# timbroed/HRFuser

Measured on AMD Instinct MI355X. Metric: train images/sec HRFuser-T r640 3-modal @1/2/4/8 MI355X; fwd ms/img, higher is better.
Workload: dtype f32; 1 GPU; t_nus_bn backbone train step (fwd+bwd+grad exchange+AdamW at lr 0), 2 img/GPU, 2x3x384x640 camera + 2 modalities, BN, single GPU; global_batch=2, parallelism=dp1, launch=hipGraph replay

## Files before the change

hrfuser_amd/_lib.py:

```python
import ctypes
import os
import re

import torch

_HERE = os.path.dirname(os.path.abspath(__file__))
HEADER = os.path.join(os.path.dirname(_HERE), 'include', 'hrfuser_hip.h')
DEBUG_HEADER = os.path.join(os.path.dirname(_HERE), 'include', 'hrfuser_hip_debug.h')
LIB_PATH = os.environ.get('HRF_LIB_PATH') or os.path.join(_HERE, 'libhrfuser_hip.so')

def _header_int(name, default):
    m = re.search(r'#define\s+' + name + r'\s+(\d+)', open(HEADER).read())
    return int(m.group(1)) if m else default


STAT_COPIES = _header_int('HRF_STAT_COPIES', 16)
FIN_MAXC = _header_int('HRF_FIN_MAXC', 576)
C3X_MAXC = _header_int('HRF_C3X_MAXC', 256)

def struct_from_header(tag, path=HEADER):
    src = re.sub(r'/\*.*?\*/', '', open(path).read(), flags=re.S)
    m = re.search(r'typedef\s+struct\s+' + tag + r'\s*\{(.*?)\}\s*' + tag + r'_t\s*;', src, flags=re.S)
    if not m:
        raise KeyError(tag)
# ... 19 lines not shown
    return type(tag, (ctypes.Structure,), {'_fields_': fields})


BnFin = struct_from_header('hrf_bn_fin')
BnBFin = struct_from_header('hrf_bn_bfin')
AttnBlock = struct_from_header('hrf_attn_block')
FfnEval = struct_from_header('hrf_ffn_eval')
Conv3xPackJob = struct_from_header('hrf_conv3x_pack_job')
P2p = struct_from_header('hrf_p2p')


def _ptr(t):
    return None if t is None else t.data_ptr()


_RAW_RETURN = ('hrf_conv3_wgrad_wide_scratch', 'hrf_conv_bwd_weight_scratch', 'hrf_conv3x_pack_size', 'hrf_conv3x_supported', 'hrf_conv_fwd_split_scratch', 'hrf_wgrad_group_report', 'hrf_attn_block_supported', 'hrf_attn_block_bwd_supported', 'hrf_group_count',
               'hrf_ffn_eval_supported', 'hrf_get_deterministic', 'hrf_det_bins_bytes', 'hrf_conv3_bf16x3_supported')
_ERR = {1: 'HRF_ERR_ARG (bad argument)', 2: 'HRF_ERR_LAUNCH (kernel launch failed)'}


class HRFuserHipError(RuntimeError):
    pass


def parse_header(path=HEADER):
    src = open(path).read()
    src = re.sub(r'/\*.*?\*/', '', src, flags=re.S)
    protos = {}
    for m in re.finditer(r'\b(?:int|long)\s+(hrf_\w+)\s*\(([^)]*)\)\s*;', src):
        args = []
        for a in m.group(2).split(','):
# ... 103 lines not shown
```

hrfuser_amd/backbone.py:

```python
import os
import warnings

import torch
import torch.nn as nn

from . import _lib
from . import runtime as R
from .registry import BACKBONES

WIN = 7


def build_bn(norm_cfg, c):
    cfg = dict(norm_cfg or dict(type='BN'))
    kind = cfg.pop('type')
    if kind not in ('BN', 'SyncBN', 'GN'):
        raise KeyError(f'unsupported norm_cfg type {kind}')
    requires_grad = cfg.pop('requires_grad', True)
    if kind == 'GN':
        if 'num_groups' not in cfg:
            raise AssertionError('norm_cfg of type GN needs num_groups')
        bn = nn.GroupNorm(cfg['num_groups'], c, eps=cfg.get('eps', 1e-5))
    else:
        bn = nn.BatchNorm2d(c, eps=cfg.get('eps', 1e-5), momentum=cfg.get('momentum', 0.1))
# ... 147 lines not shown
            od += 4 * C * K
            of += 7 * C
            oc += C
        self._csum = csum
        self._rs0 = bns[0].running_mean.data_ptr() if (bns and bns[0].running_mean is not None) else 0
        if bns:
            self._gidx, self._bidx = torch.cat(gidx).to(device), torch.cat(bidx).to(device)
            self._epsv = torch.cat(epsv).to(device)
        offs = {id(p): o for p, (o, _) in zip(params, self._spans)}
        self._poffs = offs
        self.fs_layers, self.fs_sig = {}, None
        self.pslot, cols, ps = {}, [], 0
        for m in self.root.modules():
            hit = isinstance(m, nn.LayerNorm) or (isinstance(m, nn.Conv2d) and m.groups == m.in_channels and m.groups > 1)
            cand = (m.weight, m.bias) if hit else ()
            if hasattr(m, 'relative_position_bias_table'):
                cand = (m.relative_position_bias_table,) + tuple(
                    getattr(m, n).bias for n in ('qkv', 'k_proj', 'v_proj') if hasattr(m, n))
            for q in cand:
                if q is None or id(q) not in offs or id(q) in self.pslot:
                    continue
                self.pslot[id(q)] = ps
                cols.append(torch.arange(offs[id(q)], offs[id(q)] + q.numel(), dtype=torch.int32))
                ps += q.numel()
        self.ps_n = ps
        self.ps_map = (torch.cat(cols) if cols else torch.zeros(0, dtype=torch.int32)).to(device)
        self.ps_scratch = torch.zeros(max(1, K * ps), device=device, dtype=torch.float32)
        self.ps_dirty = False
        nbt = [m.num_batches_tracked for m in bns if m.num_batches_tracked is not None]
        self.nbt_flat = torch.zeros(len(nbt), device=device, dtype=torch.long)
# ... 1555 lines not shown
```

hrfuser_amd/csrc/conv_engine.hip:

```cpp
#include <algorithm>
#include <cstdlib>
#include <vector>
#include "hrf_common.h"
#include "hrf_group.h"
#include "hrf_lin.h"
#include "../../include/hrfuser_hip.h"

#include "hrf_wgrad.h"

namespace {

constexpr int BM = 64;
constexpr int BK = 64;
constexpr int LDK = 65;
constexpr float SENT = -1.0e30f;

static int g_knob[12] = {0, 0, 0, 0, 0, 0, 0, 0, 0, 0, 0, 0};

__device__ __forceinline__ float act_at_read(int tf, float u) {
  return tf == HRF_TF_AFFINE_RELU ? fmaxf(u, 0.f) : (tf == HRF_TF_AFFINE_GELU ? hrf_gelu(u) : u);
}

struct ConvFwdArgs {
  const float* x; const float* w; const float* bias;
// ... 922 lines not shown
  if (KH == 3 && stride == 2 && Cout >= (g_knob[5] > 0 ? g_knob[5] : 16) && sC == 1 && sY == W * sX && sB == H * sY && g_knob[6] == 0) {
    Conv3Args c{};
    c.in = dy + doff; c.ldIn = ldD; c.in2 = cA != nullptr ? yraw + doff : nullptr; c.t0 = cA; c.t1 = cB; c.t2 = cC;
    c.w = w; c.wCin = Cin; c.out = dx; c.ldOut = sX; c.accumulate = accumulate; c.epi = epi; c.xraw = xraw; c.ldXr = ldXr;
    c.esc = tf_scale; c.esh = tf_shift; c.act = act; c.stats = stats; c.bfin = a.bfin;
    c.B = B; c.H = H; c.W = W; c.Cin = Cout; c.Cout = Cin; c.Hs = a.Ho; c.Ws = a.Wo;
    return hrf_conv3s2_bwd_data_launch(c, stream);
  }
  const int nt = pick_nt(Cin);
  if (KH == 1) {
    if (cA != nullptr) { HRF_BD_NT(1, true) } else { HRF_BD_NT(1, false) }
  } else {
    if (cA != nullptr) { HRF_BD_NT(3, true) } else { HRF_BD_NT(3, false) }
  }
  return hrf_check_launch();
}

extern "C" int hrf_conv3x_supported(int Cin, int Cout, int KH, int stride, int dir) {
  if (KH != 3 || Cin <= 0 || Cout <= 0) return 0;
  if (dir == 0) return (stride == 1 || stride == 2) && Cout > 32 ? 1 : 0;
  if (stride == 2) return Cin > 32 && Cout <= 64 ? 1 : 0;
  return stride == 1 && Cin > 32 ? 1 : 0;
}

extern "C" int hrf_conv_fwd_packed(const float* x, int sB, int sY, int sX, int sC, int B, int H, int W, int Cin,
                                   const float* w, const float* bias, int KH, int stride, int Cout,
                                   float* y, int ldY, int yoff, const float* res, const float* res2, int ldR,
                                   int tf_mode, const float* tf_scale, const float* tf_shift,
                                   const float* tf_rowstat, double* stats, const hrf_bn_fin_t* tf_fin, float* ln_rowstat,
                                   float ln_eps, const float* wp, void* stream) {
// ... 335 lines not shown
```

hrfuser_amd/csrc/hrf_lin.h:

```cpp
#pragma once
#include "../../include/hrfuser_hip.h"

struct LinFwdArgs {
  const float* x; int ldX;
  const float* w; const float* bias;
  float* y; int ldY; int yoff;
  const float* res; const float* res2; int ldR;
  int tf_mode; const float* tf_scale; const float* tf_shift; const float* tf_rowstat;
  double* stats;
  float* ln_out; float ln_eps;
  hrf_bn_fin_t fin;
  int M, K, N;
};

struct LinBwdDataArgs {
  const float* dy; int ldD; int doff; const float* yraw;
  const float* cA; const float* cB; const float* cC;
  const float* w;
  float* dx; int ldDx; int accumulate;
  int epi; const float* xraw; int ldXr; const float* tf_scale; const float* tf_shift; int act;
  double* stats;
  hrf_bn_bfin_t bfin;
  int M, K, N;
};

int hrf_lin_fwd_launch(const LinFwdArgs& a, void* stream);
bool hrf_lin_fwd_emits_ln(const LinFwdArgs& a);
int hrf_lin_bwd_data_launch(const LinBwdDataArgs& a, void* stream);
int hrf_lin2_fwd_launch(const LinFwdArgs& a, void* stream);
bool hrf_lin2_fwd_emits_ln(const LinFwdArgs& a);
int hrf_lin2_bwd_data_launch(const LinBwdDataArgs& a, void* stream);

struct Conv3Args {
  const float* in; int ldIn;
  const float* in2;
  const float* t0; const float* t1; const float* t2;
  int tf_mode;
  const float* w; int wCin;
  const float* bias;
  float* out; int ldOut; int ooff;
  const float* res; const float* res2; int ldR;
  int accumulate, epi; const float* xraw; int ldXr; const float* esc; const float* esh; int act;
  double* stats;
  hrf_bn_fin_t fin;
  hrf_bn_bfin_t bfin;
  int B, H, W, Cin, Cout;
// ... 31 lines not shown
```

hrfuser_amd/csrc/lin2_engine.hip:

```cpp
#include <type_traits>
#include "hrf_common.h"
#include "hrf_lin.h"
#include "hrf_group.h"
#include "../../include/hrfuser_hip.h"

namespace {

constexpr int GK = 16, GLP = GK + 4, NW = 4, NTHR = 64 * NW, GROWS = 16 * NW;

template <int CG_, int CT_, int PD_>
struct Tile {
  static constexpr int CG = CG_, CT = CT_, PD = PD_;
  static constexpr int NB = CG * CT * 16, RT = CG, RG = NW / CG;
  static constexpr int SLOT = (GROWS + NB) * GLP;
  static constexpr int NWV = (NB * 4 + NTHR - 1) / NTHR;
  static constexpr int Q = CT * 4, PE = CT * 16 + 4, NRG = NTHR / Q, NR = (GROWS + NRG - 1) / NRG;
  static constexpr int RED = NRG * 2 * CT * 16;
  static_assert(GROWS * PE <= 2 * SLOT, "the transposed accumulator tile must fit the operand ring");
};
typedef Tile<1, 5, 4> TileA;
typedef Tile<2, 5, 4> TileB;
typedef Tile<2, 8, 2> TileC;
typedef Tile<2, 10, 2> TileD;

// ... 574 lines not shown

int hrf_lin2_fwd_launch(const LinFwdArgs& a, void* stream) {
  if (!wide_enough(a.M, a.K, a.N)) return -1;
  if (a.ln_out != nullptr && g_l2_knob[0] != 1) return -1;
  if ((long)a.M * a.ldX >= (1L << 32)) return -1;
  if (a.tf_mode != HRF_TF_NONE && a.tf_mode != HRF_TF_LN && a.fin.stats != nullptr && a.K > HRF_FIN_MAXC) return -1;
  const int id = pick_tile(a.N);
  switch (id) {
    case 1: return launch_fwd_tf<TileA>(a, id, stream);
    case 2: return launch_fwd_tf<TileB>(a, id, stream);
    case 3: return launch_fwd_tf<TileC>(a, id, stream);
    default: return launch_fwd_tf<TileD>(a, id, stream);
  }
}
bool hrf_lin2_fwd_emits_ln(const LinFwdArgs&) { return false; }
int hrf_lin2_bwd_data_launch(const LinBwdDataArgs& a, void* stream) {
  if (!wide_enough(a.M, a.K, a.N)) return -1;
  if (a.cA != nullptr && a.bfin.gstats != nullptr && a.K > HRF_FIN_MAXC) return -1;
  if ((long)a.M * a.ldD + a.doff >= (1L << 32)) return -1;
  const int id = pick_tile(a.N);
  switch (id) {
    case 1: return launch_bwd_b<TileA>(a, id, stream);
    case 2: return launch_bwd_b<TileB>(a, id, stream);
    case 3: return launch_bwd_b<TileC>(a, id, stream);
    default: return launch_bwd_b<TileD>(a, id, stream);
  }
}
#if defined(HRF_L2_TIMING) && !defined(HRF_EMUL)
extern "C" int hrf_lin2_stamps(long long* out) {
  return hipMemcpyFromSymbol(out, HIP_SYMBOL(g_l2_t), sizeof(long long) * 64) == hipSuccess ? HRF_OK : HRF_ERR_LAUNCH;
// ... 8 lines not shown
```

hrfuser_amd/csrc/lin_engine.hip:

```cpp
#include "hrf_common.h"
#include "hrf_lin.h"
#include "hrf_group.h"
#include "../../include/hrfuser_hip.h"

namespace {

#ifndef HRF_LIN_BWD_EPI_MAX_NT
#define HRF_LIN_BWD_EPI_MAX_NT 5
#endif
constexpr int LIN_BWD_EPI_MAX_NT = HRF_LIN_BWD_EPI_MAX_NT;
#ifndef HRF_LIN_FWD_MAX_NT
#define HRF_LIN_FWD_MAX_NT 5
#endif
constexpr int LIN_FWD_MAX_NT = HRF_LIN_FWD_MAX_NT;
constexpr int LIN_SB = 3, LIN_SB_WIDE = 2, LIN_SB_WIDE_K = 64;

__device__ float g_zero4[4] = {0.f, 0.f, 0.f, 0.f};

template <bool V4>
__device__ __forceinline__ hrf_f4 ld_group(const float* p, long off, int nvalid) {
  if (V4) return hrf_ld4(nvalid > 0 ? p + off : g_zero4);
  hrf_f4 r;
#pragma unroll
  for (int e = 0; e < 4; ++e) r[e] = *(e < nvalid ? p + off + e : g_zero4);
// ... 157 lines not shown
    float sq = 0.f;
#pragma unroll
    for (int t = 0; t < NT; ++t)
#pragma unroll
      for (int r = 0; r < 4; ++r) { const float dd = (16 * t + 4 * q + r < a.N) ? acc[t][r] - mu : 0.f; sq = fmaf(dd, dd, sq); }
    sq += __shfl_xor(sq, 16); sq += __shfl_xor(sq, 32);
    if (q == 0 && pixv) { a.ln_out[2 * (long)pix] = mu; a.ln_out[2 * (long)pix + 1] = 1.0f / sqrtf(sq / (float)a.N + a.ln_eps); }
  }
  if (a.stats != nullptr) {
    wave_moments<NT>(sStat, wave, j, q, pixv, n0w, a.N, acc, acc);
    __syncthreads();
    flush_moments<NT>(sStat, a.stats, n0w, a.N);
  }
}

template <int NT, bool BNB, int SB, bool SK, bool ONE = false>
__global__ __launch_bounds__(256) void lin_bwd_data_kernel(HrfGroup<LinBwdDataArgs> grp) {
  const LinBwdDataArgs& a = grp.sel();
  __shared__ float sStat[4 * 2 * NT * 16];
  __shared__ __attribute__((aligned(16))) float sRed[SK ? 3 * NT * 256 : 4];
  __shared__ __attribute__((aligned(16))) float sFin[BNB ? 3 * HRF_FIN_MAXC : 4];
  const int tid = threadIdx.x, lane = tid & 63, wave = tid >> 6;
  const int j = lane & 15, q = lane >> 4;
  const int n0w = blockIdx.y * (NT * 16);
  const int pix = SK ? blockIdx.x * 16 + j : blockIdx.x * 64 + wave * 16 + j;
  const bool pixin = pix < a.M;
  const bool pixv = pixin && (!SK || wave == 0);
  const long pc = pixin ? pix : a.M - 1;
  const float* cAp = a.cA;
  const float* cBp = a.cB;
  const float* cCp = a.cC;
  if (BNB) {
    if (a.bfin.gstats != nullptr) {
      hrf_bn_bfin_onload(a.bfin, sFin, sFin + HRF_FIN_MAXC, sFin + 2 * HRF_FIN_MAXC, tid, 256, blockIdx.x == 0 && blockIdx.y == 0);
      __syncthreads();
      cAp = sFin; cBp = sFin + HRF_FIN_MAXC; cCp = sFin + 2 * HRF_FIN_MAXC;
    }
  }

  hrf_f4 acc[NT], xr[NT];
#pragma unroll
  for (int t = 0; t < NT; ++t) {
    const int chb = n0w + 16 * t + 4 * q, nval = a.N - chb;
    const bool nfull = n0w + 16 * (t + 1) <= a.N;
    xr[t] = ld_sel(nfull, a.xraw, pc * a.ldXr + chb, a.epi == 1 ? nval : 0);
    acc[t] = ld_sel(nfull, a.dx, pc * a.ldDx + chb, (a.epi != 1 && a.accumulate && (!SK || wave == 0)) ? nval : 0);
  }

  const int nslab = (a.K + 15) >> 4;
  const int kper = SK ? (nslab + 3) >> 2 : nslab;
  const int k0 = SK ? wave * kper : 0, k1 = SK ? min(nslab, k0 + kper) : nslab;
  const long drow = pc * a.ldD + a.doff;
#pragma unroll 1
  for (int kb = k0; kb < (ONE ? k0 + 1 : k1); kb += SB) {
    hrf_f4 dv[SB], yv[SB], ca[SB], cb[SB], cc[SB], wv[SB][NT];
#pragma unroll
    for (int s = 0; s < SB; ++s) {
      const int kbase = 16 * (kb + s) + 4 * q, kval = (!SK || kb + s < k1) ? a.K - kbase : 0;
      const bool kfull = 16 * (kb + s + 1) <= a.K;
      dv[s] = ld_sel(kfull, a.dy, drow + kbase, kval);
      if (BNB) {
        yv[s] = ld_sel(kfull, a.yraw, drow + kbase, kval);
        ca[s] = ld_sel(kfull, cAp, kbase, kval); cb[s] = ld_sel(kfull, cBp, kbase, kval); cc[s] = ld_sel(kfull, cCp, kbase, kval);
// ... 1 lines not shown
#pragma unroll
      for (int t = 0; t < NT; ++t) {
        const int ci = n0w + 16 * t + j;
#pragma unroll
        for (int r = 0; r < 4; ++r)
          wv[s][t][r] = *((r < kval && ci < a.N) ? a.w + (long)(kbase + r) * a.N + ci : g_zero4);
      }
    }
#pragma unroll
    for (int s = 0; s < SB; ++s) {
#pragma unroll
      for (int r = 0; r < 4; ++r) {
        const float d = BNB ? fmaf(ca[s][r], dv[s][r], fmaf(cb[s][r], yv[s][r], cc[s][r])) : dv[s][r];
#pragma unroll
        for (int t = 0; t < NT; ++t) acc[t] = hrf_mfma16(wv[s][t][r], d, acc[t]);
      }
    }
  }
  if (SK) {
    if (wave != 0) {
#pragma unroll
      for (int t = 0; t < NT; ++t) hrf_st4(sRed + (((wave - 1) * NT + t) * 64 + lane) * 4, acc[t]);
    }
    __syncthreads();
    if (wave == 0) {
#pragma unroll
      for (int w = 0; w < 3; ++w)
#pragma unroll
        for (int t = 0; t < NT; ++t) {
          const hrf_f4 v = hrf_ld4(sRed + ((w * NT + t) * 64 + lane) * 4);
// ... 128 lines not shown
      case 1: HRF_LB_ONE(1, BNB_) break;                 \
      case 2: HRF_LB_ONE(2, BNB_) break;                 \
      case 3: HRF_LB_ONE(3, BNB_) break;                 \
      case 5: HRF_LB_ONE(5, BNB_) break;                 \
      default: HRF_LB_ONE(5, BNB_) break;                \
    }                                                    \
  } else                                                 \
  switch (ntw) {                                         \
    case 1: HRF_LB_LAUNCH(1, BNB_, LIN_SB, SK_); break;  \
    case 2: HRF_LB_LAUNCH(2, BNB_, LIN_SB, SK_); break;  \
    case 3: HRF_LB_LAUNCH(3, BNB_, LIN_SB, SK_); break;  \
    default: HRF_LB_WIDE(5, BNB_, SK_) break;            \
  }
#define HRF_LB_V4(BNB_) { if (sk) { HRF_LB_NT(BNB_, true) } else { HRF_LB_NT(BNB_, false) } }

int hrf_lin_bwd_data_launch(const LinBwdDataArgs& a, void* stream) {
  if (a.K < 4 || a.N < 4 || a.M <= 0) return -1;
  const int T = (a.N + 15) / 16;
  const bool sk = T <= 9 && lin_use_sk(a.M, a.K);
  int ntw = pick_ntw(sk ? 4 * a.M : a.M, T);
  if (ntw > LIN_BWD_EPI_MAX_NT) ntw = LIN_BWD_EPI_MAX_NT;
  const dim3 grid(hrf_cdiv(a.M, sk ? 16 : 64), hrf_cdiv(T, ntw));
  if (a.cA != nullptr) { HRF_LB_V4(true) } else { HRF_LB_V4(false) }
  return hrf_check_launch();
}
```

hrfuser_amd/profiling.py:

```python
import ctypes
import math
import os
import time

import torch

from . import _lib
from .runtime import gc_paused as _gc_paused


def _pick_nt(C):
    T = (C + 15) // 16
    best, cost = 2, 1 << 30
    for nt in (2, 3, 4):
        c = ((T + nt - 1) // nt) * nt
        if c <= cost:
            cost, best = c, nt
    return best


def _out_hw(H, W, KH, s):
    p = KH // 2
    return (H + 2 * p - KH) // s + 1, (W + 2 * p - KH) // s + 1

# ... 8 lines not shown
            return 'conv3x_kernel<0, 2>', 2.0 * M * a['Cout'] * K, by
        if a['KH'] == 1 and a['stride'] == 1 and a['sC'] == 1 and a['Cin'] >= 4 and a['Cout'] >= 4:
            return 'lin_fwd_kernel', 2.0 * M * a['Cout'] * K, by
        return f"conv_fwd_kernel<{_pick_nt(a['Cout'])},{a['KH']},{a['tf_mode']}>", 2.0 * M * a['Cout'] * K, by
    if name in ('hrf_conv_bwd_data', 'hrf_conv_bwd_data_packed'):
        Ho, Wo = _out_hw(a['H'], a['W'], a['KH'], a['stride'])
        M, K = a['B'] * a['H'] * a['W'], a['KH'] ** 2 * a['Cout']
        by = f4 * (a['B'] * Ho * Wo * a['Cout'] * (2 if a['cA'] is not None else 1) + a['Cin'] * K
                   + M * a['Cin'] * (2 if a['epi'] else 1 + bool(a['accumulate'])))
        fl = 2.0 * a['B'] * Ho * Wo * a['Cin'] * K
        if name == 'hrf_conv_bwd_data_packed':
            return f"conv3x_kernel<{a['stride']}, 2>", fl, by
        if a['KH'] == 1 and a['stride'] == 1 and a['sC'] == 1 and a['Cin'] >= 4 and a['Cout'] >= 4:
            return 'lin_bwd_data_kernel', fl, by
        return f"conv_bwd_data_kernel<{_pick_nt(a['Cin'])},{a['KH']},{int(a['cA'] is not None)}>", fl, by
    if name == 'hrf_conv_bwd_weight_s':
        Ho, Wo = _out_hw(a['H'], a['W'], a['KH'], a['stride'])
        Mp, Np = a['B'] * Ho * Wo, a['KH'] ** 2 * a['Cin']
        by = f4 * (Mp * a['Cout'] * (2 if a['cA'] is not None else 1) + a['B'] * a['H'] * a['W'] * a['Cin'] + a['Cout'] * Np)
        return f"wgrad3x_kernel<{a['stride']}>", 2.0 * Mp * a['Cout'] * Np, by
    if name == 'hrf_conv_bwd_weight':
        Ho, Wo = _out_hw(a['H'], a['W'], a['KH'], a['stride'])
        Mp, Np = a['B'] * Ho * Wo, a['KH'] ** 2 * a['Cin']
        by = f4 * (Mp * a['Cout'] * (2 if a['cA'] is not None else 1) + a['B'] * a['H'] * a['W'] * a['Cin'] + a['Cout'] * Np)
        dense = a['sC'] == 1 and (a['KH'] == 3 or a['stride'] == 1)
        return ('wgrad_dense_kernel' if dense else 'conv_bwd_wgt_kernel'), 2.0 * Mp * a['Cout'] * Np, by
    if name in ('hrf_dwconv_fwd', 'hrf_dwconv_bwd_weight'):
        Ho, Wo = _out_hw(a['H'], a['W'], 3, a['stride'])
        n_in, n_out = a['B'] * a['H'] * a['W'] * a['C'], a['B'] * Ho * Wo * a['C']
        if name == 'hrf_dwconv_fwd':
# ... 669 lines not shown
```

hrfuser_amd/runtime.py:

```python
import ctypes
import os

import torch

try:
    import greenlet as _greenlet
except Exception:
    _greenlet = None

from . import _lib

_DW_FUSED_WG = os.environ.get('HRF_DW_FUSED_WG', '1') != '0'
_FIN_ONLOAD = os.environ.get('HRF_FIN_ONLOAD', '1') != '0'
_XHUB = os.environ.get('HRF_XHUB', '0') != '0'
_LANE_COMMS = os.environ.get('HRF_SYNC_LANE_COMMS', '0') == '1'


def _p2p_mode_id():
    from . import p2p
    return {'off': 0, 'on': 1, 'auto': 2}[p2p.mode()]


def set_lane_comms(on):
    global _LANE_COMMS
# ... 237 lines not shown
class Strand:
    __slots__ = ('lane', 'tape', 'glet', 'pending', 'wait', 'parent', 'kids_alive', 'cur')

    def __init__(self, lane, parent=None):
        self.lane, self.parent = lane, parent
        self.tape = []
        self.glet = None
        self.pending = None
        self.wait = None
        self.kids_alive = 0
        self.cur = lane


_GROUPABLE = frozenset((
    'hrf_conv_fwd', 'hrf_conv_bwd_data', 'hrf_conv_fwd_packed', 'hrf_conv_bwd_data_packed', 'hrf_dwconv_fwd', 'hrf_dwconv_bwd_data',
    'hrf_dwconv_bwd_data_weight',
    'hrf_attn_block_fwd', 'hrf_attn_block_bwd', 'hrf_affine_act_res', 'hrf_act_bwd', 'hrf_scale_add', 'hrf_ln_stats',
    'hrf_ln_bwd', 'hrf_window_attn_fwd', 'hrf_window_attn_bwd', 'hrf_fuse_sum', 'hrf_bilinear_up_bwd'))
_NO_PARK = frozenset(_lib._RAW_RETURN) | frozenset((
    'hrf_wgrad_group_begin', 'hrf_wgrad_group_end', 'hrf_group_begin', 'hrf_group_end', 'hrf_debug_knob'))


class _LibProxy:

    def __init__(self, ctx, lib):
        self.__dict__['_ctx'] = ctx
        self.__dict__['_lib'] = lib

    def __getattr__(self, name):
        fn = getattr(self.__dict__['_lib'], name)
        if name in _NO_PARK:
# ... 486 lines not shown

    def run_backward(self):
        eng = self.owner._engine()
        if getattr(self, 'gen', None) is not None and self.gen != getattr(eng, 'gen', self.gen):
            raise _lib.HRFuserHipError(
                'backward of a forward pass that is no longer the latest one of this module: every forward re-uses the '
                'BatchNorm statistics slots and step buffers of its engine, so `net(x1); net(x2); loss.backward()` would '
                'back-propagate x1 with the statistics of x2.  Run backward before the next forward of the same module '
                '(or use two module instances).')
        if self.det != bool(self.lib.hrf_get_deterministic()):
            raise _lib.HRFuserHipError('backward of a forward pass that ran in the other deterministic mode: the moment slots '
                                       'of the forward hold ' + ('integer bins' if self.det else 'doubles') + ' the backward '
                                       'kernels would misread (set_deterministic between forward and backward)')
        if self.det:
            eng.det_begin()
        use_keep_list(self.owner._engine().keep)
        self.owner._engine().fs_prepare()
        self._flush_n = int(os.environ.get('HRF_WGRAD_FLUSH', '48')) if (self.multi and os.environ.get('HRF_WGRAD', 'defer') == 'flush') else 0
        entry = torch.cuda.current_stream() if self.multi else None
        if self.multi:
            self.main.stream.wait_stream(entry)
        self.strand = self.root
        self._run_tape(self.root)
        if self._deferred and os.environ.get('HRF_DEBUG_SKIP_WGRAD') == '1':
            self._deferred = []
        eng0 = self.owner._engine()
        if eng0.rpb_pending():
            if self._deferred:
                self._deferred.append((eng0.fs_rpb_bytes, lambda: eng0.rpb_grad_now(self.L, self.stream), None, None))
            else:
# ... 300 lines not shown
                                    P(cC), st.count, 1 if st.train else 0, 1, st.C)
    local = None
    if coll:
        local = _keep(st.gstats.clone())
        ctx.all_reduce(st.gstats)
    ctx.L.hrf_bn_bwd_finalize(st.gstats, local, st.bn.weight, st.mean, st.invstd, st.count, 1 if st.train else 0,
                              wg, bg, cA, cB, cC, st.C, ctx.stream)
    return st.coef, None


def _conv_out_hw(H, W, KH, stride):
    pad = KH // 2
    return (H + 2 * pad - KH) // stride + 1, (W + 2 * pad - KH) // stride + 1


_S2F_MINPIX = int(os.environ.get('HRF_C3X_S2F_MINPIX', '4096'))
_IM2COL = os.environ.get('HRF_IM2COL', '1') != '0'


def _packed(ctx, weight, direction, strides, B, H, W, Cin, coef_channels=0):
    if coef_channels > _lib.C3X_MAXC:
        return None
    eng = ctx.owner._engine()
    wp = eng.packed(weight, direction) if hasattr(eng, 'packed') else None
    if wp is None or tuple(strides) != (H * W * Cin, W * Cin, Cin, 1):
        return None
    return wp


def _conv_backward(ctx, src, weight, bias, KH, stride, Cout, dy, ldD, doff, yraw, st=None):
# ... 5 lines not shown

    def bwd_data(*args):
        if wpb is not None:
            L.hrf_conv_bwd_data_packed(*args[:-1], wpb, args[-1])
        else:
            L.hrf_conv_bwd_data(*args)
    bfin = None
    cA = cB = cC = None
    if st is not None:
        (cA, cB, cC), bfin = bn_backward_coef(ctx, st, consumer_follows=needs)
    if not needs:
        pass
    elif isinstance(src, Lazy):
        ps = src.st
        ps.du = _new_like(ps.raw)
        bwd_data(dy, ldD, doff, yraw, cA, cB, cC, bfin, weight, KH, stride, Cout, B, H, W, Cin,
                            ps.du, *strides, 0, 1, ps.raw, Cin, ps.scale, ps.shift, _TF2ACT[src.mode],
                            ps.gstats, s)
    elif isinstance(src, LNIn):
        da = _new_like(src.act.t)
        bwd_data(dy, ldD, doff, yraw, cA, cB, cC, bfin, weight, KH, stride, Cout, B, H, W, Cin,
                            da, *strides, 0, 0, None, 0, None, None, 0, None, s)
        g, acc = src.act.grad_target()
        eng = ctx.owner._engine()
        gacc, cs = eng.grad_acc(src.ln.weight)
        bacc, _ = eng.grad_acc(src.ln.bias)
        L.hrf_ln_bwd(da, src.act.t, src.rowstat, src.ln.weight, B * H * W, Cin, g, acc, gacc, bacc, cs, s)
    elif isinstance(src, Act):
        g, acc = src.grad_target()
        bwd_data(dy, ldD, doff, yraw, cA, cB, cC, bfin, weight, KH, stride, Cout, B, H, W, Cin,
# ... 182 lines not shown
        mask, mscale, rowscale = drop
        y = _new_like(res.t)
        L.hrf_conv_fwd(o.t, *strides, B, H, W, C, w, b, 1, 1, C, y, C, 0, None, None, 0,
                       TF_NONE, None, None, None, None, None, None, 0.0, s)
        L.hrf_scale_add(y, mask, mscale, rowscale, H * W, res.t, res2.t if res2 is not None else None,
                        out.t, rows, C, s)

    def bwd():
        g = out.grad
        if drop is None:
            dy = g
        else:
            mask, mscale, rowscale = drop
            dy = _new_like(g)
            L.hrf_scale_add(g, mask, mscale, rowscale, H * W, None, None, dy, rows, C, s)
        if w.requires_grad:
            L.hrf_conv_bwd_weight(dy, C, 0, None, None, None, None, o.t, *strides, B, H, W, C, 1, 1, C,
                                  TF_NONE, None, None, None, w.grad, b.grad if b is not None else None, s)
        og, acc = o.grad_target()
        L.hrf_conv_bwd_data(dy, C, 0, None, None, None, None, None, w, 1, 1, C, B, H, W, C, og, *strides, acc,
                            0, None, 0, None, None, 0, None, s)
        if res2 is not None and res2.needs_grad:
            if res2.grad is None and res.grad is None and res.needs_grad:
                res2.grad = gpu_clone(g)
            else:
                res2.add_grad(g)
        if res.needs_grad:
            res.add_grad(g)
    ctx.push(bwd)
    return out


def ln_input(ctx, act, ln, cache=None):
    B, H, W, C = act.t.shape
    key = (id(act), float(ln.eps))
    pre = getattr(act, 'rowstat', None)
# ... 393 lines not shown
```

include/hrfuser_hip.h:

```cpp
#ifndef HRFUSER_HIP_H_
#define HRFUSER_HIP_H_

#ifndef HRF_STAT_COPIES
#define HRF_STAT_COPIES 4
#endif

#define HRF_FIN_MAXC 576
#define HRF_C3X_MAXC 256
typedef struct hrf_bn_fin {
  const double* stats;
  const float* gamma; const float* beta; float* running_mean; float* running_var;
  float* scale; float* shift; float* mean; float* invstd;
  double count; float eps; float momentum; int update_running; int write; int C;
  int copies;
  const double* count_ptr;
} hrf_bn_fin_t;
typedef struct hrf_bn_bfin {
  const double* gstats;
  const float* gamma; const float* mean; const float* invstd;
  float* dgamma; float* dbeta; float* cA; float* cB; float* cC;
  double count; int train; int write; int C;
  int copies;
  const double* gstats_local;
  float pgrad_scale;
// ... 12 lines not shown
long hrf_conv_fwd_split_scratch(int sB, int sY, int sX, int sC, int B, int H, int W, int Cin, int KH, int stride, int Cout,
                                int ldY, int yoff);
int hrf_conv_fwd_split(const float* x, int sB, int sY, int sX, int sC, int B, int H, int W, int Cin,
                       const float* w, const float* bias, int KH, int stride, int Cout,
                       float* y, int ldY, int yoff, const float* res, const float* res2, int ldR,
                       int tf_mode, const float* tf_scale, const float* tf_shift,
                       const float* tf_rowstat, double* stats, const hrf_bn_fin_t* tf_fin, float* ln_rowstat, float ln_eps,
                       float* scratch, void* stream);
int hrf_conv_bwd_data(const float* dy, int ldD, int doff, const float* yraw,
                      const float* cA, const float* cB, const float* cC, const hrf_bn_bfin_t* bfin,
                      const float* w, int KH, int stride, int Cout,
                      int B, int H, int W, int Cin,
                      float* dx, int sB, int sY, int sX, int sC, int accumulate,
                      int epi, const float* xraw, int ldXr, const float* tf_scale,
                      const float* tf_shift, int act, double* stats, void* stream);
int hrf_conv_bwd_weight(const float* dy, int ldD, int doff, const float* yraw,
                        const float* cA, const float* cB, const float* cC,
                        const float* x, int sB, int sY, int sX, int sC,
                        int B, int H, int W, int Cin, int KH, int stride, int Cout,
                        int tf_mode, const float* tf_scale, const float* tf_shift,
                        const float* tf_rowstat, float* dw, float* dbias, void* stream);

typedef struct hrf_conv3x_pack_job {
  const float* w; float* wp;
  int Cout, Cin, dir;
} hrf_conv3x_pack_job_t;
long hrf_conv3x_pack_size(int Cout, int Cin, int dir);
int hrf_conv3x_pack(const hrf_conv3x_pack_job_t* jobs, int n, void* stream);
int hrf_conv3x_supported(int Cin, int Cout, int KH, int stride, int dir);
int hrf_conv_fwd_packed(const float* x, int sB, int sY, int sX, int sC, int B, int H, int W, int Cin,
// ... 206 lines not shown
```

Before: 186.6 images/sec.

## Fuse 1x1 conv weight-gradient into the backward-data linear kernel

Adds a WG variant of lin_bwd_data_kernel that also computes the weight and bias gradients from the same dy tile while producing dx. An MFMA outer product is built from LDS-transposed x and dy, and the partials are merged across waves or atomically added into per-copy gradient buffers. By default it is used for attention projection 1x1 convs with small row counts. This saves a separate bwd_weight launch and a second read of dy and x. In exchange it adds atomics and LDS reduction traffic, and it moves some CrossFFN output-layer params into a different grad-accumulation group.

```diff
diff --git a/hrfuser_amd/_lib.py b/hrfuser_amd/_lib.py
--- a/hrfuser_amd/_lib.py
+++ b/hrfuser_amd/_lib.py
@@ -57,7 +57,7 @@
     return None if t is None else t.data_ptr()
 
 
-_RAW_RETURN = ('hrf_conv3_wgrad_wide_scratch', 'hrf_conv_bwd_weight_scratch', 'hrf_conv3x_pack_size', 'hrf_conv3x_supported', 'hrf_conv_fwd_split_scratch', 'hrf_wgrad_group_report', 'hrf_attn_block_supported', 'hrf_attn_block_bwd_supported', 'hrf_group_count',
+_RAW_RETURN = ('hrf_conv3_wgrad_wide_scratch', 'hrf_conv_bwd_weight_scratch', 'hrf_conv3x_pack_size', 'hrf_conv3x_supported', 'hrf_conv_bwd_data_weight_supported', 'hrf_conv_fwd_split_scratch', 'hrf_wgrad_group_report', 'hrf_attn_block_supported', 'hrf_attn_block_bwd_supported', 'hrf_group_count',
                'hrf_ffn_eval_supported', 'hrf_get_deterministic', 'hrf_det_bins_bytes', 'hrf_conv3_bf16x3_supported')
 _ERR = {1: 'HRF_ERR_ARG (bad argument)', 2: 'HRF_ERR_LAUNCH (kernel launch failed)'}
 
diff --git a/hrfuser_amd/backbone.py b/hrfuser_amd/backbone.py
--- a/hrfuser_amd/backbone.py
+++ b/hrfuser_amd/backbone.py
@@ -185,6 +185,8 @@
         for m in self.root.modules():
             hit = isinstance(m, nn.LayerNorm) or (isinstance(m, nn.Conv2d) and m.groups == m.in_channels and m.groups > 1)
             cand = (m.weight, m.bias) if hit else ()
+            if isinstance(m, CrossFFN) and m.layers[6].out_channels <= 48:
+                cand = (m.layers[6].weight, m.layers[6].bias)
             if hasattr(m, 'relative_position_bias_table'):
                 cand = (m.relative_position_bias_table,) + tuple(
                     getattr(m, n).bias for n in ('qkv', 'k_proj', 'v_proj') if hasattr(m, n))
diff --git a/hrfuser_amd/csrc/conv_engine.hip b/hrfuser_amd/csrc/conv_engine.hip
--- a/hrfuser_amd/csrc/conv_engine.hip
+++ b/hrfuser_amd/csrc/conv_engine.hip
@@ -960,6 +960,44 @@
     if (cA != nullptr) { HRF_BD_NT(3, true) } else { HRF_BD_NT(3, false) }
   }
   return hrf_check_launch();
+}
+
+extern "C" int hrf_conv_bwd_data_weight_supported(int Cin, int Cout, long rows, int epi, int bnb) {
+  if (Cin <= 0 || Cout <= 0 || rows <= 0 || (epi != 0 && epi != 1) || g_knob[4] != 0) return 0;
+  if (rows > (1L << 30)) return 0;
+  if (hrf_lin2_bwd_data_wide(rows, Cout, Cin)) return 0;
+  return hrf_lin_bwd_data_wg_ok((int)rows, Cout, Cin, bnb != 0) ? 1 : 0;
+}
+
+extern "C" int hrf_conv_bwd_data_weight(const float* dy, int ldD, int doff, const float* yraw,
+                                        const float* cA, const float* cB, const float* cC, const hrf_bn_bfin_t* bfin,
+                                        const float* w, int KH, int stride, int Cout,
+                                        int B, int H, int W, int Cin,
+                                        float* dx, int sB, int sY, int sX, int sC, int accumulate,
+                                        int epi, const float* xraw, int ldXr, const float* tf_scale,
+                                        const float* tf_shift, int act, double* stats,
+                                        const float* x, int ldX, float* dw, float* dbias, long copy_stride, void* stream) {
+  HRF_GROUP_CALL();
+  if (KH != 1 || stride != 1 || !(sC == 1 && sX == Cin && sY == W * sX && sB == H * sY)) return HRF_ERR_ARG;
+  if (bfin != nullptr && (cA == nullptr || bfin->C != Cout || Cout > HRF_FIN_MAXC || bfin->gstats == nullptr)) return HRF_ERR_ARG;
+  if (dy == nullptr || w == nullptr || dx == nullptr || dw == nullptr || copy_stride < 0) return HRF_ERR_ARG;
+  if (epi == 1 ? (xraw == nullptr || tf_scale == nullptr || tf_shift == nullptr || ldXr < Cin) : (x == nullptr || ldX < Cin)) return HRF_ERR_ARG;
+  const long rows = (long)B * H * W;
+  if (rows <= 0 || !hrf_conv_bwd_data_weight_supported(Cin, Cout, rows, epi, cA != nullptr ? 1 : 0)) return HRF_ERR_ARG;
+  if (!hrf_det_fin_ok(bfin)) return HRF_ERR_ARG;
+  bool det_ok = true;
+  dw = hrf_det_grad(dw, det_ok); dbias = hrf_det_grad(dbias, det_ok);
+  if (!det_ok) return HRF_ERR_ARG;
+  LinBwdDataArgs l;
+  l.bfin = hrf_bn_bfin_t{};
+  if (bfin != nullptr) l.bfin = *bfin;
+  l.dy = dy; l.ldD = ldD; l.doff = doff; l.yraw = yraw; l.cA = cA; l.cB = cB; l.cC = cC; l.w = w;
+  l.dx = dx; l.ldDx = sX; l.accumulate = accumulate; l.epi = epi; l.xraw = xraw; l.ldXr = ldXr;
+  l.tf_scale = tf_scale; l.tf_shift = tf_shift; l.act = act; l.stats = hrf_det_tag(stats);
+  l.M = (int)rows; l.K = Cout; l.N = Cin;
+  l.x = x; l.ldX = ldX; l.dw = dw; l.dbias = dbias; l.copy_stride = copy_stride;
+  const int rc = hrf_lin_bwd_data_launch(l, stream);
+  return rc >= 0 ? rc : HRF_ERR_ARG;
 }
 
 extern "C" int hrf_conv3x_supported(int Cin, int Cout, int KH, int stride, int dir) {
diff --git a/hrfuser_amd/csrc/hrf_lin.h b/hrfuser_amd/csrc/hrf_lin.h
--- a/hrfuser_amd/csrc/hrf_lin.h
+++ b/hrfuser_amd/csrc/hrf_lin.h
@@ -22,14 +22,18 @@
   double* stats;
   hrf_bn_bfin_t bfin;
   int M, K, N;
+  const float* x = nullptr; int ldX = 0;
+  float* dw = nullptr; float* dbias = nullptr; long copy_stride = 0;
 };
 
 int hrf_lin_fwd_launch(const LinFwdArgs& a, void* stream);
 bool hrf_lin_fwd_emits_ln(const LinFwdArgs& a);
 int hrf_lin_bwd_data_launch(const LinBwdDataArgs& a, void* stream);
+bool hrf_lin_bwd_data_wg_ok(int M, int K, int N, bool bnb);
 int hrf_lin2_fwd_launch(const LinFwdArgs& a, void* stream);
 bool hrf_lin2_fwd_emits_ln(const LinFwdArgs& a);
 int hrf_lin2_bwd_data_launch(const LinBwdDataArgs& a, void* stream);
+bool hrf_lin2_bwd_data_wide(long M, int K, int N);
 
 struct Conv3Args {
   const float* in; int ldIn;
diff --git a/hrfuser_amd/csrc/lin2_engine.hip b/hrfuser_amd/csrc/lin2_engine.hip
--- a/hrfuser_amd/csrc/lin2_engine.hip
+++ b/hrfuser_amd/csrc/lin2_engine.hip
@@ -612,6 +612,7 @@
   }
 }
 bool hrf_lin2_fwd_emits_ln(const LinFwdArgs&) { return false; }
+bool hrf_lin2_bwd_data_wide(long M, int K, int N) { return wide_enough(M, K, N); }
 int hrf_lin2_bwd_data_launch(const LinBwdDataArgs& a, void* stream) {
   if (!wide_enough(a.M, a.K, a.N)) return -1;
   if (a.cA != nullptr && a.bfin.gstats != nullptr && a.K > HRF_FIN_MAXC) return -1;
diff --git a/hrfuser_amd/csrc/lin_engine.hip b/hrfuser_amd/csrc/lin_engine.hip
--- a/hrfuser_amd/csrc/lin_engine.hip
+++ b/hrfuser_amd/csrc/lin_engine.hip
@@ -195,12 +195,15 @@
   }
 }
 
-template <int NT, bool BNB, int SB, bool SK, bool ONE = false>
+constexpr int LIN_WG_LD = 20;
+template <int NT, bool BNB, int SB, bool SK, bool ONE = false, bool WG = false>
 __global__ __launch_bounds__(256) void lin_bwd_data_kernel(HrfGroup<LinBwdDataArgs> grp) {
   const LinBwdDataArgs& a = grp.sel();
   __shared__ float sStat[4 * 2 * NT * 16];
   __shared__ __attribute__((aligned(16))) float sRed[SK ? 3 * NT * 256 : 4];
   __shared__ __attribute__((aligned(16))) float sFin[BNB ? 3 * HRF_FIN_MAXC : 4];
+  __shared__ __attribute__((aligned(16))) float sTr[WG ? 4 * 16 * LIN_WG_LD : 4];
+  __shared__ __attribute__((aligned(16))) float sMrg[(WG && !SK) ? 2 * (4 * NT * 256 + 64) : 4];
   const int tid = threadIdx.x, lane = tid & 63, wave = tid >> 6;
   const int j = lane & 15, q = lane >> 4;
   const int n0w = blockIdx.y * (NT * 16);
@@ -228,6 +231,46 @@
     acc[t] = ld_sel(nfull, a.dx, pc * a.ldDx + chb, (a.epi != 1 && a.accumulate && (!SK || wave == 0)) ? nval : 0);
   }
 
+  hrf_f4 xb[WG ? NT : 1];
+  float* const sT = sTr + (WG ? wave * 16 * LIN_WG_LD : 0);
+  const long wcp = WG ? (long)(blockIdx.x % HRF_STAT_COPIES) * a.copy_stride : 0;
+  int mbuf = 0;
+  if (WG) {
+    hrf_f4 xv[NT];
+#pragma unroll
+    for (int t = 0; t < NT; ++t) {
+      const int chb = n0w + 16 * t + 4 * q, nval = a.N - chb;
+      const bool nfull = n0w + 16 * (t + 1) <= a.N;
+      if (a.epi == 1) {
+        const hrf_f4 esc = ld_sel(nfull, a.tf_scale, chb, nval), esh = ld_sel(nfull, a.tf_shift, chb, nval);
+#pragma unroll
+        for (int r = 0; r < 4; ++r) xv[t][r] = fmaf(xr[t][r], esc[r], esh[r]);
+      } else {
+        xv[t] = ld_sel(nfull, a.x, pc * a.ldX + chb, nval);
+      }
+    }
+    if (a.epi == 1) {
+      hrf_with_act(a.act, [&](auto kind) HRF_KIND_INLINE {
+        constexpr int ACT = decltype(kind)::value;
+#pragma unroll
+        for (int t = 0; t < NT; ++t)
+#pragma unroll
+          for (int r = 0; r < 4; ++r) xv[t][r] = hrf_act(ACT, xv[t][r]);
+      });
+    }
+#pragma unroll
+    for (int t = 0; t < NT; ++t) {
+#pragma unroll
+      for (int r = 0; r < 4; ++r) {
+        const bool cv = n0w + 16 * t + 4 * q + r < a.N;
+        sT[(4 * q + r) * LIN_WG_LD + j] = (pixin && cv) ? xv[t][r] : 0.f;
+      }
+      HRF_WAVE_SYNC();
+      xb[t] = hrf_ld4(sT + j * LIN_WG_LD + 4 * q);
+      HRF_WAVE_SYNC();
+    }
+  }
+
   const int nslab = (a.K + 15) >> 4;
   const int kper = SK ? (nslab + 3) >> 2 : nslab;
   const int k0 = SK ? wave * kper : 0, k1 = SK ? min(nslab, k0 + kper) : nslab;
@@ -259,6 +302,69 @@
         const float d = BNB ? fmaf(ca[s][r], dv[s][r], fmaf(cb[s][r], yv[s][r], cc[s][r])) : dv[s][r];
 #pragma unroll
         for (int t = 0; t < NT; ++t) acc[t] = hrf_mfma16(wv[s][t][r], d, acc[t]);
+      }
+    }
+    if (WG) {
+#pragma unroll
+      for (int s = 0; s < SB; ++s) {
+        const int slab = kb + s;
+        if (slab < k1) {
+          float bs[4];
+#pragma unroll
+          for (int r = 0; r < 4; ++r) {
+            const float d = BNB ? fmaf(ca[s][r], dv[s][r], fmaf(cb[s][r], yv[s][r], cc[s][r])) : dv[s][r];
+            const float dm = (pixin && 16 * slab + 4 * q + r < a.K) ? d : 0.f;
+            sT[(4 * q + r) * LIN_WG_LD + j] = dm;
+            bs[r] = hrf_row16_sum(dm);
+          }
+          HRF_WAVE_SYNC();
+          const hrf_f4 da = hrf_ld4(sT + j * LIN_WG_LD + 4 * q);
+          HRF_WAVE_SYNC();
+          hrf_f4 wacc[NT];
+#pragma unroll
+          for (int t = 0; t < NT; ++t) wacc[t] = hrf_f4{0.f, 0.f, 0.f, 0.f};
+#pragma unroll
+          for (int m = 0; m < 4; ++m)
+#pragma unroll
+            for (int t = 0; t < NT; ++t) wacc[t] = hrf_mfma16(da[m], xb[t][m], wacc[t]);
+          if (SK) {
+#pragma unroll
+            for (int t = 0; t < NT; ++t)
+#pragma unroll
+              for (int r = 0; r < 4; ++r) {
+                const int k = 16 * slab + 4 * q + r, ci = n0w + 16 * t + j;
+                if (k < a.K && ci < a.N) hrf_grad_add(a.dw, wcp, (long)k * a.N + ci, wacc[t][r]);
+              }
+            if (a.dbias != nullptr && blockIdx.y == 0 && j == 0) {
+#pragma unroll
+              for (int r = 0; r < 4; ++r)
+                if (16 * slab + 4 * q + r < a.K) hrf_grad_add(a.dbias, wcp, 16 * slab + 4 * q + r, bs[r]);
+            }
+          } else {
+            float* const sM = sMrg + mbuf * (4 * NT * 256 + 64);
+#pragma unroll
+            for (int t = 0; t < NT; ++t)
+#pragma unroll
+              for (int r = 0; r < 4; ++r) sM[wave * (NT * 256) + (t * 4 + r) * 64 + lane] = wacc[t][r];
+            if (j == 0) {
+#pragma unroll
+              for (int r = 0; r < 4; ++r) sM[4 * NT * 256 + wave * 16 + 4 * q + r] = bs[r];
+            }
+            __syncthreads();
+#pragma unroll
+            for (int t = 0; t < NT; ++t) {
+              const int idx = t * 256 + tid;
+              const float v = (sM[idx] + sM[NT * 256 + idx]) + (sM[2 * NT * 256 + idx] + sM[3 * NT * 256 + idx]);
+              const int k = 16 * slab + 4 * q + wave, ci = n0w + 16 * t + j;
+              if (k < a.K && ci < a.N) hrf_grad_add(a.dw, wcp, (long)k * a.N + ci, v);
+            }
+            if (a.dbias != nullptr && blockIdx.y == 0 && tid < 16 && 16 * slab + tid < a.K) {
+              const float* b = sM + 4 * NT * 256;
+              hrf_grad_add(a.dbias, wcp, 16 * slab + tid, (b[tid] + b[16 + tid]) + (b[32 + tid] + b[48 + tid]));
+            }
+            mbuf ^= 1;
+          }
+        }
       }
     }
   }
@@ -417,13 +523,45 @@
   }
 #define HRF_LB_V4(BNB_) { if (sk) { HRF_LB_NT(BNB_, true) } else { HRF_LB_NT(BNB_, false) } }
 
+#define HRF_LBW(NT_, BNB_, SB_, SK_, ONE_) HRF_LAUNCH_G((lin_bwd_data_kernel<NT_, BNB_, SB_, SK_, ONE_, true>), grid, dim3(256), 0, stream, a)
+#define HRF_LBW_ONE(NT_)                                           \
+  { if (a.K <= 16) { HRF_LBW(NT_, true, 1, false, true); }         \
+    else if (a.K <= 32) { HRF_LBW(NT_, true, 2, false, true); }    \
+    else { HRF_LBW(NT_, true, 3, false, true); } }
+#define HRF_LBW_WIDE(SK_) { if (a.K <= LIN_SB_WIDE_K) { HRF_LBW(5, false, LIN_SB, SK_, false); } else { HRF_LBW(5, false, LIN_SB_WIDE, SK_, false); } }
+#define HRF_LBW_NT(SK_)                                    \
+  switch (ntw) {                                           \
+    case 1: HRF_LBW(1, false, LIN_SB, SK_, false); break;  \
+    case 2: HRF_LBW(2, false, LIN_SB, SK_, false); break;  \
+    case 3: HRF_LBW(3, false, LIN_SB, SK_, false); break;  \
+    default: HRF_LBW_WIDE(SK_) break;                      \
+  }
+constexpr int LIN_WG_MAX_K = 160;
+bool hrf_lin_bwd_data_wg_ok(int M, int K, int N, bool bnb) {
+  if (K < 4 || N < 4 || M <= 0 || K > LIN_WG_MAX_K) return false;
+  return K <= 48 ? bnb : !bnb;
+}
+static int lin_bwd_data_wg_launch(const LinBwdDataArgs& a, int ntw, bool sk, dim3 grid, void* stream) {
+  if (a.K <= 48) {
+    switch (ntw) {
+      case 1: HRF_LBW_ONE(1) break;
+      case 2: HRF_LBW_ONE(2) break;
+      case 3: HRF_LBW_ONE(3) break;
+      default: HRF_LBW_ONE(5) break;
+    }
+  } else if (sk) { HRF_LBW_NT(true) } else { HRF_LBW_NT(false) }
+  return hrf_check_launch();
+}
+
 int hrf_lin_bwd_data_launch(const LinBwdDataArgs& a, void* stream) {
   if (a.K < 4 || a.N < 4 || a.M <= 0) return -1;
+  if (a.dw != nullptr && !hrf_lin_bwd_data_wg_ok(a.M, a.K, a.N, a.cA != nullptr)) return -1;
   const int T = (a.N + 15) / 16;
   const bool sk = T <= 9 && lin_use_sk(a.M, a.K);
   int ntw = pick_ntw(sk ? 4 * a.M : a.M, T);
   if (ntw > LIN_BWD_EPI_MAX_NT) ntw = LIN_BWD_EPI_MAX_NT;
   const dim3 grid(hrf_cdiv(a.M, sk ? 16 : 64), hrf_cdiv(T, ntw));
+  if (a.dw != nullptr) return lin_bwd_data_wg_launch(a, ntw, sk, grid, stream);
   if (a.cA != nullptr) { HRF_LB_V4(true) } else { HRF_LB_V4(false) }
   return hrf_check_launch();
 }
diff --git a/hrfuser_amd/profiling.py b/hrfuser_amd/profiling.py
--- a/hrfuser_amd/profiling.py
+++ b/hrfuser_amd/profiling.py
@@ -46,6 +46,11 @@
         if a['KH'] == 1 and a['stride'] == 1 and a['sC'] == 1 and a['Cin'] >= 4 and a['Cout'] >= 4:
             return 'lin_bwd_data_kernel', fl, by
         return f"conv_bwd_data_kernel<{_pick_nt(a['Cin'])},{a['KH']},{int(a['cA'] is not None)}>", fl, by
+    if name == 'hrf_conv_bwd_data_weight':
+        M = a['B'] * a['H'] * a['W']
+        by = f4 * (M * a['Cout'] * (2 if a['cA'] is not None else 1) + 2 * a['Cin'] * a['Cout']
+                   + M * a['Cin'] * (2 if a['epi'] else 2 + bool(a['accumulate'])))
+        return 'lin_bwd_data_kernel', 4.0 * M * a['Cin'] * a['Cout'], by
     if name == 'hrf_conv_bwd_weight_s':
         Ho, Wo = _out_hw(a['H'], a['W'], a['KH'], a['stride'])
         Mp, Np = a['B'] * Ho * Wo, a['KH'] ** 2 * a['Cin']
diff --git a/hrfuser_amd/runtime.py b/hrfuser_amd/runtime.py
--- a/hrfuser_amd/runtime.py
+++ b/hrfuser_amd/runtime.py
@@ -275,7 +275,7 @@
 
 _GROUPABLE = frozenset((
     'hrf_conv_fwd', 'hrf_conv_bwd_data', 'hrf_conv_fwd_packed', 'hrf_conv_bwd_data_packed', 'hrf_dwconv_fwd', 'hrf_dwconv_bwd_data',
-    'hrf_dwconv_bwd_data_weight',
+    'hrf_dwconv_bwd_data_weight', 'hrf_conv_bwd_data_weight',
     'hrf_attn_block_fwd', 'hrf_attn_block_bwd', 'hrf_affine_act_res', 'hrf_act_bwd', 'hrf_scale_add', 'hrf_ln_stats',
     'hrf_ln_bwd', 'hrf_window_attn_fwd', 'hrf_window_attn_bwd', 'hrf_fuse_sum', 'hrf_bilinear_up_bwd'))
 _NO_PARK = frozenset(_lib._RAW_RETURN) | frozenset((
@@ -792,6 +792,7 @@
                                        'kernels would misread (set_deterministic between forward and backward)')
         if self.det:
             eng.det_begin()
+        self.lin_fused = lin_fused_sites()
         use_keep_list(self.owner._engine().keep)
         self.owner._engine().fs_prepare()
         self._flush_n = int(os.environ.get('HRF_WGRAD_FLUSH', '48')) if (self.multi and os.environ.get('HRF_WGRAD', 'defer') == 'flush') else 0
@@ -1122,6 +1123,28 @@
     return (H + 2 * pad - KH) // stride + 1, (W + 2 * pad - KH) // stride + 1
 
 
+_LIN_FUSED_WG_DEFAULT = 'proj'
+_LIN_FUSED_MAX_ROWS_PLAIN = 2048
+
+
+def lin_fused_sites(value=None):
+    v = (os.environ.get('HRF_LIN_FUSED_WG', _LIN_FUSED_WG_DEFAULT) if value is None else value).strip().lower()
+    if v not in ('0', 'proj', 'ffn', 'all'):
+        raise ValueError(f"HRF_LIN_FUSED_WG={v!r}: one of 0, proj, ffn, all")
+    return {'0': frozenset(), 'proj': frozenset(('proj',)), 'ffn': frozenset(('ffn',)), 'all': frozenset(('proj', 'ffn'))}[v]
+
+
+def _lin_fused(ctx, site, Cin, Cout, rows, epi, bnb, copy_stride):
+    sites = ctx.__dict__.get('lin_fused')
+    if sites is None:
+        sites = lin_fused_sites()
+    if site not in sites or not hasattr(ctx.L, 'hrf_conv_bwd_data_weight'):
+        return False
+    if copy_stride == 0 and rows > _LIN_FUSED_MAX_ROWS_PLAIN:
+        return False
+    return bool(ctx.L.hrf_conv_bwd_data_weight_supported(Cin, Cout, rows, epi, 1 if bnb else 0))
+
+
 _S2F_MINPIX = int(os.environ.get('HRF_C3X_S2F_MINPIX', '4096'))
 _IM2COL = os.environ.get('HRF_IM2COL', '1') != '0'
 
@@ -1157,6 +1180,17 @@
     elif isinstance(src, Lazy):
         ps = src.st
         ps.du = _new_like(ps.raw)
+        fused = False
+        if KH == 1 and stride == 1 and weight.requires_grad and tuple(strides) == _nhwc_strides(B, H, W, Cin):
+            eng = ctx.owner._engine()
+            wacc, cs = eng.grad_acc(weight)
+            bacc, bcs = eng.grad_acc(bias) if (bias is not None and bias.requires_grad) else (None, cs)
+            fused = bcs == cs and _lin_fused(ctx, 'ffn', Cin, Cout, B * H * W, 1, cA is not None, cs)
+        if fused:
+            L.hrf_conv_bwd_data_weight(dy, ldD, doff, yraw, cA, cB, cC, bfin, weight, KH, stride, Cout, B, H, W, Cin,
+                                       ps.du, *strides, 0, 1, ps.raw, Cin, ps.scale, ps.shift, _TF2ACT[src.mode],
+                                       ps.gstats, None, 0, wacc, bacc, cs, s)
+            return
         bwd_data(dy, ldD, doff, yraw, cA, cB, cC, bfin, weight, KH, stride, Cout, B, H, W, Cin,
                             ps.du, *strides, 0, 1, ps.raw, Cin, ps.scale, ps.shift, _TF2ACT[src.mode],
                             ps.gstats, s)
@@ -1369,12 +1403,16 @@
             mask, mscale, rowscale = drop
             dy = _new_like(g)
             L.hrf_scale_add(g, mask, mscale, rowscale, H * W, None, None, dy, rows, C, s)
-        if w.requires_grad:
-            L.hrf_conv_bwd_weight(dy, C, 0, None, None, None, None, o.t, *strides, B, H, W, C, 1, 1, C,
-                                  TF_NONE, None, None, None, w.grad, b.grad if b is not None else None, s)
         og, acc = o.grad_target()
-        L.hrf_conv_bwd_data(dy, C, 0, None, None, None, None, None, w, 1, 1, C, B, H, W, C, og, *strides, acc,
-                            0, None, 0, None, None, 0, None, s)
+        if w.requires_grad and _lin_fused(ctx, 'proj', C, C, rows, 0, False, 0):
+            L.hrf_conv_bwd_data_weight(dy, C, 0, None, None, None, None, None, w, 1, 1, C, B, H, W, C, og, *strides, acc,
+                                       0, None, 0, None, None, 0, None, o.t, C, w.grad, b.grad if b is not None else None, 0, s)
+        else:
+            if w.requires_grad:
+                L.hrf_conv_bwd_weight(dy, C, 0, None, None, None, None, o.t, *strides, B, H, W, C, 1, 1, C,
+                                      TF_NONE, None, None, None, w.grad, b.grad if b is not None else None, s)
+            L.hrf_conv_bwd_data(dy, C, 0, None, None, None, None, None, w, 1, 1, C, B, H, W, C, og, *strides, acc,
+                                0, None, 0, None, None, 0, None, s)
         if res2 is not None and res2.needs_grad:
             if res2.grad is None and res.grad is None and res.needs_grad:
                 res2.grad = gpu_clone(g)
diff --git a/include/hrfuser_hip.h b/include/hrfuser_hip.h
--- a/include/hrfuser_hip.h
+++ b/include/hrfuser_hip.h
@@ -50,6 +50,15 @@
                       float* dx, int sB, int sY, int sX, int sC, int accumulate,
                       int epi, const float* xraw, int ldXr, const float* tf_scale,
                       const float* tf_shift, int act, double* stats, void* stream);
+int hrf_conv_bwd_data_weight_supported(int Cin, int Cout, long rows, int epi, int bnb);
+int hrf_conv_bwd_data_weight(const float* dy, int ldD, int doff, const float* yraw,
+                             const float* cA, const float* cB, const float* cC, const hrf_bn_bfin_t* bfin,
+                             const float* w, int KH, int stride, int Cout,
+                             int B, int H, int W, int Cin,
+                             float* dx, int sB, int sY, int sX, int sC, int accumulate,
+                             int epi, const float* xraw, int ldXr, const float* tf_scale,
+                             const float* tf_shift, int act, double* stats,
+                             const float* x, int ldX, float* dw, float* dbias, long copy_stride, void* stream);
 int hrf_conv_bwd_weight(const float* dy, int ldD, int doff, const float* yraw,
                         const float* cA, const float* cB, const float* cC,
                         const float* x, int sB, int sY, int sX, int sC,
```

After: 188.6 images/sec, median of 6. 1.01x the previous value.
